# DeNA/HandyRL

Measured on NVIDIA H100. Metric: learner_samples_per_sec, higher is better.
Workload: dtype fp32

## Files before the change

handyrl_b200/csrc/gemm_kernel.cu:

```cuda
#include <cuda_runtime.h>
#include <stdint.h>
#include <string.h>

#define HRL_GEMM_KERNEL gemm_tf32x3_kernel
#define HRL_GEMM_BF16 false
#include "gemm_common.cuh"

static int g_gemm_debug = 0;
extern "C" void hrl_gemm_set_debug(int v) { g_gemm_debug = v; }

namespace hrl {

__global__ void sum_partials_kernel(const float *__restrict__ partials, int splits, long long n, long long stride, float *__restrict__ out) {
    for (long long i = (long long)blockIdx.x * blockDim.x + threadIdx.x; i < n; i += (long long)gridDim.x * blockDim.x) {
        float s = partials[i];
        for (int k = 1; k < splits; k++) s += partials[(long long)k * stride + i];
        out[i] = s;
    }
}

template <bool A_K, bool B_K, bool PACKED, int NW>
static int launch_gemm(const GemmParams &p, dim3 grid, size_t smem_bytes, cudaStream_t stream) {
    HRL_CUDA_CHECK(cudaFuncSetAttribute(gemm_tf32x3_kernel<A_K, B_K, PACKED, NW>, cudaFuncAttributeMaxDynamicSharedMemorySize, (int)smem_bytes));
    gemm_tf32x3_kernel<A_K, B_K, PACKED, NW><<<grid, kGemmThreads, smem_bytes, stream>>>(p);
    return HRL_OK;
}

template <int NW>
static int launch_gemm_width(const GemmParams &p, dim3 grid, size_t smem_bytes, cudaStream_t stream) {
    if (p.b.packed) return p.a.kmajor ? launch_gemm<true, true, true, NW>(p, grid, smem_bytes, stream)
                                      : launch_gemm<false, true, true, NW>(p, grid, smem_bytes, stream);
    if (p.a.kmajor) return p.b.kmajor ? launch_gemm<true, true, false, NW>(p, grid, smem_bytes, stream)
                                      : launch_gemm<true, false, false, NW>(p, grid, smem_bytes, stream);
    return p.b.kmajor ? launch_gemm<false, true, false, NW>(p, grid, smem_bytes, stream)
                      : launch_gemm<false, false, false, NW>(p, grid, smem_bytes, stream);
}

}


extern "C" size_t hrl_gemm_workspace_floats(int64_t M, int64_t N, int64_t K, int32_t splits) {
    (void)K;
    return splits > 1 ? (size_t)splits * (size_t)M * (size_t)N : 0;
}

extern "C" int32_t hrl_gemm_effective_splits(int64_t K, int32_t splits) {
    const int total_chunks = (int)((K + hrl::kChunkK - 1) / hrl::kChunkK);
    if (splits < 1) splits = 1;
    if (splits > total_chunks) splits = total_chunks;
    const int per = (total_chunks + splits - 1) / splits;
    return (total_chunks + per - 1) / per;
}

extern "C" int hrl_gemm_fused(const HrlGemmArgs *args, void *stream_) {
    using namespace hrl;
    cudaStream_t stream = reinterpret_cast<cudaStream_t>(stream_);
    HRL_REQUIRE(args != nullptr, HRL_ERR_BAD_ARG, "hrl_gemm_fused: args is NULL");
    const HrlGemmArgs &g = *args;
    const int64_t M = g.M, N = g.N, K = g.K;
    int splits = g.splits;
    HRL_REQUIRE(g.a.ptr && g.b.ptr && (g.C || ((splits > 1 || g.segments > 0) && g.workspace)), HRL_ERR_BAD_ARG, "hrl_gemm_fused: NULL pointer");
    HRL_REQUIRE(M > 0 && N > 0 && K > 0 && M < (1ll << 31) && N < (1ll << 22) && K < (1ll << 31) && g.b.ld < (1ll << 22), HRL_ERR_BAD_ARG,
                "hrl_gemm_fused: bad dimensions (M=%lld N=%lld K=%lld)", (long long)M, (long long)N, (long long)K);
    HRL_REQUIRE(g.conv_mode >= 0 && g.conv_mode <= 2, HRL_ERR_BAD_ARG, "hrl_gemm_fused: conv_mode is 0, 1 or 2");
    if (g.conv_mode != 0) {
        HRL_REQUIRE(g.conv_off && g.conv_hw > 0 && g.conv_taps > 0 && g.conv_cin > 0 && g.conv_cin < 65536 &&
                        (long long)g.conv_hw * g.conv_taps <= hrl::kConvMaxTable && g.a.p == nullptr && g.b.p == nullptr && g.splits >= 1,
                    HRL_ERR_BAD_ARG, "hrl_gemm_fused: convolution geometry (at most 256 cells x 9 taps, plain operands)");
        if (g.conv_mode == 1)
            HRL_REQUIRE(g.b.packed && g.a.kmajor && g.a.ld >= g.conv_cin && g.a.ld % 4 == 0 && (reinterpret_cast<uintptr_t>(g.a.ptr) & 15) == 0 &&
                            M % g.conv_hw == 0 && K == (int64_t)g.conv_taps * ((g.conv_cin + kChunkK - 1) / kChunkK) * kChunkK && g.splits == 1,
                        HRL_ERR_UNSUPPORTED,
                        "hrl_gemm_fused: convolution forward needs a packed B image over taps x (channels padded to 32), 16-byte aligned "
                        "pixel rows and whole boards");
        else
            HRL_REQUIRE(!g.b.packed && !g.a.kmajor && !g.b.kmajor && g.b.ld >= g.conv_cin &&
                            N == (int64_t)g.conv_taps * g.conv_cin + (g.conv_ones_row ? 1 : 0) && K % g.conv_hw == 0,
                        HRL_ERR_UNSUPPORTED,
                        "hrl_gemm_fused: convolution weight gradient reduces over whole boards of pixels, N = taps x channels (+ 1 with the ones row)");
    }
    HRL_REQUIRE(g.segments >= 0 && g.segments <= hrl::kMaxSegments &&
                    (g.segments == 0 || (g.conv_mode == 2 && g.seg_a && g.seg_b && g.workspace && g.C == nullptr)),
                HRL_ERR_BAD_ARG, "hrl_gemm_fused: up to %d segments, of a convolution weight gradient left as slice partials in the workspace",
                hrl::kMaxSegments);
    HRL_REQUIRE(!g.conv_ones_row || g.conv_mode == 2, HRL_ERR_BAD_ARG, "hrl_gemm_fused: the ones row belongs to the convolution weight gradient");
    HRL_REQUIRE((g.conv_mode == 1 || g.a.ld >= (g.a.kmajor ? K : M)) && (g.b.packed || g.conv_mode == 2 || g.b.ld >= (g.b.kmajor ? K : N)) &&
                    (g.C == nullptr || g.ldc >= N),
                HRL_ERR_BAD_ARG, "hrl_gemm_fused: leading dimension smaller than the row length");
    HRL_REQUIRE(!g.a.packed && (!g.b.packed || (N <= hrl::kMaxN && g.b.p == nullptr && (reinterpret_cast<uintptr_t>(g.b.ptr) & 15) == 0)),
                HRL_ERR_BAD_ARG, "hrl_gemm_fused: only an untransformed B operand of at most 288 rows can be a packed image");
    HRL_REQUIRE((g.a.p == nullptr) == (g.a.r == nullptr) && (g.b.p == nullptr) == (g.b.r == nullptr) &&
                    (g.a.ptr2 == nullptr || (g.a.p && g.a.q)) && (g.b.ptr2 == nullptr || (g.b.p && g.b.q)),
                HRL_ERR_BAD_ARG, "hrl_gemm_fused: an operand transform needs p and r (and q with a second source)");
    HRL_REQUIRE(g.epilogue >= HRL_GEMM_EP_STORE && g.epilogue <= HRL_GEMM_EP_MASK_STATS, HRL_ERR_BAD_ARG, "hrl_gemm_fused: unknown epilogue");
    HRL_REQUIRE(g.epilogue != HRL_GEMM_EP_MASK_STATS || (g.ep_y != nullptr && g.ep_ldy >= N && (g.ep_mean == nullptr) == (g.ep_rstd == nullptr)),
                HRL_ERR_BAD_ARG, "hrl_gemm_fused: the masked epilogue needs the pre-activation tile");
    HRL_REQUIRE(g.epilogue < HRL_GEMM_EP_STATS || (N % 4 == 0 && g.ldc % 4 == 0 && (reinterpret_cast<uintptr_t>(g.C) & 15) == 0 && g.col_partials),
                HRL_ERR_UNSUPPORTED, "hrl_gemm_fused: the statistics epilogues need N and ldc multiples of 4, a 16-byte aligned C and col_partials");
    const int total_chunks = (int)((K + kChunkK - 1) / kChunkK);
    if (splits < 1) splits = 1;
    if (splits > total_chunks) splits = total_chunks;
    HRL_REQUIRE((splits == 1 && g.segments == 0) || (g.workspace != nullptr && g.bias == nullptr && g.epilogue == HRL_GEMM_EP_STORE), HRL_ERR_WORKSPACE,
                "hrl_gemm_fused: a split-K product needs a workspace of hrl_gemm_workspace_floats() floats, no bias and the plain epilogue");
    const int n_tiles = (int)((N + kMaxN - 1) / kMaxN);
    const int n_widest = (int)(N < kMaxN ? N : kMaxN);
    int n_pad = (n_widest + 15) / 16 * 16;
    if (n_pad > 256) n_pad = (n_pad + 31) / 32 * 32;

    GemmParams p;
    auto operand = [](const HrlGemmOperand &o) {
        GemmOperand r;
        r.ptr = o.ptr; r.ptr2 = o.ptr2; r.p = o.p; r.q = o.q; r.r = o.r; r.ld = o.ld;
        r.kmajor = o.kmajor ? 1 : 0; r.relu = o.relu ? 1 : 0; r.feature_is_row = o.feature_is_row ? 1 : 0; r.packed = o.packed ? 1 : 0;
        return r;
    };
    p.a = operand(g.a);
    p.b = operand(g.b);
    p.bias = g.bias;
    p.M = (int)M; p.N = (int)N; p.K = (int)K;
    p.chunks_per_split = (total_chunks + splits - 1) / splits;
    p.epilogue = g.epilogue;
    p.ep_y = g.ep_y; p.ep_ldy = g.ep_ldy;
    p.ep_scale = g.ep_scale; p.ep_shift = g.ep_shift; p.ep_mean = g.ep_mean; p.ep_rstd = g.ep_rstd;
    p.col_partials = g.col_partials;
    p.debug = g_gemm_debug & 63;
    p.conv_off = g.conv_off; p.conv_mode = g.conv_mode; p.conv_hw = g.conv_hw; p.conv_taps = g.conv_taps; p.conv_cin = g.conv_cin;
    p.conv_cpt = (g.conv_cin + kChunkK - 1) / kChunkK;
    splits = (total_chunks + p.chunks_per_split - 1) / p.chunks_per_split;
    p.seg_splits = 0;
    p.conv_ones = g.conv_ones_row ? 1 : 0;
    if (g.segments > 0) {
        p.seg_splits = splits;
        for (int i = 0; i < g.segments; i++) { p.seg_a[i] = g.seg_a[i]; p.seg_b[i] = g.seg_b[i]; }
        splits *= g.segments;
    }
    if (splits > 1 || g.segments > 0) {
        p.C = g.workspace; p.ldc = N; p.c_split_stride = M * N;
    } else {
        p.C = g.C; p.ldc = g.ldc; p.c_split_stride = 0;
    }
    size_t smem_bytes = 1024 + (size_t)kStages * (g.bf16 ? ((size_t)n_pad + kTileM) * kChunkK * 2
                                                         : 2 * (size_t)n_pad * kChunkK * 4 + 2 * (size_t)kTileM * kChunkK * 4);
    const size_t red_rows = (size_t)kGemmThreads / (size_t)((n_pad - 12) / 4 > 0 ? (n_pad - 12) / 4 : 1);
    const size_t ep_bytes = 1024 + ((size_t)kTileM * (n_pad + 4) + 2 * red_rows * (size_t)n_pad) * 4;
    if (smem_bytes < ep_bytes) smem_bytes = ep_bytes;
    const dim3 grid((unsigned)((M + kTileM - 1) / kTileM), (unsigned)n_tiles, (unsigned)splits);
    int st;
    if (g.bf16) st = launch_gemm_bf16(p, n_pad / 2, grid, smem_bytes, stream);
    else switch (n_pad / 2) {
    case 8: st = launch_gemm_width<8>(p, grid, smem_bytes, stream); break;
    case 16: st = launch_gemm_width<16>(p, grid, smem_bytes, stream); break;
    case 24: st = launch_gemm_width<24>(p, grid, smem_bytes, stream); break;
    case 32: st = launch_gemm_width<32>(p, grid, smem_bytes, stream); break;
    case 40: st = launch_gemm_width<40>(p, grid, smem_bytes, stream); break;
    case 48: st = launch_gemm_width<48>(p, grid, smem_bytes, stream); break;
    case 56: st = launch_gemm_width<56>(p, grid, smem_bytes, stream); break;
    case 64: st = launch_gemm_width<64>(p, grid, smem_bytes, stream); break;
    case 72: st = launch_gemm_width<72>(p, grid, smem_bytes, stream); break;
    case 80: st = launch_gemm_width<80>(p, grid, smem_bytes, stream); break;
    case 88: st = launch_gemm_width<88>(p, grid, smem_bytes, stream); break;
    case 96: st = launch_gemm_width<96>(p, grid, smem_bytes, stream); break;
    case 104: st = launch_gemm_width<104>(p, grid, smem_bytes, stream); break;
    case 112: st = launch_gemm_width<112>(p, grid, smem_bytes, stream); break;
    case 120: st = launch_gemm_width<120>(p, grid, smem_bytes, stream); break;
    case 128: st = launch_gemm_width<128>(p, grid, smem_bytes, stream); break;
    case 144: st = launch_gemm_width<144>(p, grid, smem_bytes, stream); break;
    default: HRL_REQUIRE(false, HRL_ERR_BAD_ARG, "hrl_gemm_fused: no kernel for a tile of %d padded columns", n_pad);
    }
    if (st != HRL_OK) return st;
    HRL_CUDA_CHECK(cudaGetLastError());
    if (splits > 1 && g.C != nullptr) {
        const long long n = (long long)M * N;
        HRL_REQUIRE(g.ldc == N, HRL_ERR_UNSUPPORTED, "hrl_gemm_fused: split-K output must be dense (ldc == N)");
        int blocks = (int)((n + 255) / 256);
        if (blocks > 1184) blocks = 1184;
        sum_partials_kernel<<<blocks, 256, 0, stream>>>(g.workspace, splits, n, n, g.C);
        HRL_CUDA_CHECK(cudaGetLastError());
    }
    return HRL_OK;
}

extern "C" int hrl_gemm_tf32x3(const float *A, int64_t lda, int32_t a_kmajor, const float *B, int64_t ldb, int32_t b_kmajor,
                               const float *bias, float *C, int64_t ldc, int64_t M, int64_t N, int64_t K, int32_t splits,
                               float *workspace, void *stream) {
    HrlGemmArgs g;
    memset(&g, 0, sizeof(g));
    g.a.ptr = A; g.a.ld = lda; g.a.kmajor = a_kmajor;
    g.b.ptr = B; g.b.ld = ldb; g.b.kmajor = b_kmajor;
    g.bias = bias; g.C = C; g.ldc = ldc; g.M = M; g.N = N; g.K = K; g.splits = splits; g.workspace = workspace;
    g.epilogue = HRL_GEMM_EP_STORE;
    return hrl_gemm_fused(&g, stream);
}
```

Measured before the change: 19.29 million.

## Add specialized 3xTF32 weight-gradient GEMM kernel with larger tiles

Adds a dedicated weight-gradient GEMM kernel for M-major operands that uses 96x288 block tiles, 48x48 warp tiles, a three-stage cp.async pipeline, and conflict-free padded shared-memory strides. It applies the fused per-feature affine/ReLU transforms while loading fragments. Eligible GEMMs (fp32, no conv mode, no segments, plain store epilogue) are routed to it instead of the generic width-templated kernel. The aim is better data reuse and tensor-core throughput on wgrad shapes, at the cost of more code paths and a single-block-per-SM launch bound that may underfill the GPU on small problems.

After: 21.87 million (median of 6 runs). 1.13x the previous value.

```diff
diff --git a/handyrl_b200/csrc/gemm_kernel.cu b/handyrl_b200/csrc/gemm_kernel.cu
--- a/handyrl_b200/csrc/gemm_kernel.cu
+++ b/handyrl_b200/csrc/gemm_kernel.cu
@@ -5,6 +5,7 @@
 #define HRL_GEMM_KERNEL gemm_tf32x3_kernel
 #define HRL_GEMM_BF16 false
 #include "gemm_common.cuh"
+#include "gemm_wgrad.cuh"
 
 static int g_gemm_debug = 0;
 extern "C" void hrl_gemm_set_debug(int v) { g_gemm_debug = v; }
@@ -146,7 +147,8 @@
     if (smem_bytes < ep_bytes) smem_bytes = ep_bytes;
     const dim3 grid((unsigned)((M + kTileM - 1) / kTileM), (unsigned)n_tiles, (unsigned)splits);
     int st;
-    if (g.bf16) st = launch_gemm_bf16(p, n_pad / 2, grid, smem_bytes, stream);
+    if (gemm_wgrad_applies(g)) st = launch_gemm_wgrad(g, p.chunks_per_split, splits, p.C, p.ldc, p.c_split_stride, p.debug, stream);
+    else if (g.bf16) st = launch_gemm_bf16(p, n_pad / 2, grid, smem_bytes, stream);
     else switch (n_pad / 2) {
     case 8: st = launch_gemm_width<8>(p, grid, smem_bytes, stream); break;
     case 16: st = launch_gemm_width<16>(p, grid, smem_bytes, stream); break;
diff --git a/handyrl_b200/csrc/gemm_wgrad.cuh b/handyrl_b200/csrc/gemm_wgrad.cuh
--- /dev/null
+++ b/handyrl_b200/csrc/gemm_wgrad.cuh
@@ -0,0 +1,13 @@
+#pragma once
+#include <cuda_runtime.h>
+
+#include "common.cuh"
+
+namespace hrl {
+
+bool gemm_wgrad_applies(const HrlGemmArgs &g);
+
+int launch_gemm_wgrad(const HrlGemmArgs &g, int chunks_per_split, int splits, float *C, long long ldc, long long c_split_stride,
+                      int debug, cudaStream_t stream);
+
+}
diff --git a/handyrl_b200/csrc/gemm_wgrad_kernel.cu b/handyrl_b200/csrc/gemm_wgrad_kernel.cu
--- /dev/null
+++ b/handyrl_b200/csrc/gemm_wgrad_kernel.cu
@@ -0,0 +1,276 @@
+#include <cuda_runtime.h>
+#include <stdint.h>
+
+#include "gemm_wgrad.cuh"
+
+namespace hrl {
+namespace {
+
+constexpr int kThreads = 384;
+constexpr int kTileM = 96, kTileN = 288;
+constexpr int kWarpM = 48, kWarpN = 48;
+constexpr int kChunk = 32;
+constexpr int kStages = 3;
+constexpr int kLdA = kTileM + 8;
+constexpr int kLdB = kTileN + 8;
+constexpr int kStageFloats = 2 * kChunk * kLdA + kChunk * kLdB;
+constexpr size_t kSmemBytes = (size_t)kStages * kStageFloats * 4;
+static_assert(kLdA % 32 == 8 && kLdB % 32 == 8, "conflict-free fragment loads need row strides == 8 (mod 32) words");
+
+struct Operand {
+    const float *ptr, *ptr2;
+    const float *p, *q, *r;
+    long long ld;
+    int relu;
+};
+
+struct Params {
+    Operand a, b;
+    float *C;
+    long long ldc, c_split_stride;
+    int M, N, K, chunks_per_split;
+    int debug;
+};
+
+template <int KIND>
+__device__ __forceinline__ float transform(float x, float y, float p, float q, float r, bool relu) {
+    if (KIND == 0) return x;
+    const float v = KIND == 2 ? fmaf(x, p, fmaf(y, q, r)) : fmaf(x, p, r);
+    return relu ? fmaxf(v, 0.f) : v;
+}
+
+__device__ __forceinline__ void split(float v, uint32_t &hi, uint32_t &lo) {
+    hi = __float_as_uint(v) & 0xFFFFE000u;
+    lo = __float_as_uint(v - __uint_as_float(hi));
+}
+
+__device__ __forceinline__ void mma_tf32(float (&d)[4], const uint32_t (&a)[4], uint32_t b0, uint32_t b1) {
+    asm("mma.sync.aligned.m16n8k8.row.col.f32.tf32.tf32.f32 {%0, %1, %2, %3}, {%4, %5, %6, %7}, {%8, %9}, {%0, %1, %2, %3};"
+        : "+f"(d[0]), "+f"(d[1]), "+f"(d[2]), "+f"(d[3])
+        : "r"(a[0]), "r"(a[1]), "r"(a[2]), "r"(a[3]), "r"(b0), "r"(b1));
+}
+
+__device__ __forceinline__ void cp_async16(uint32_t dst, const float *src) {
+    asm volatile("cp.async.cg.shared.global [%0], [%1], 16;" ::"r"(dst), "l"(src) : "memory");
+}
+__device__ __forceinline__ void cp_async_commit() { asm volatile("cp.async.commit_group;" ::: "memory"); }
+template <int N>
+__device__ __forceinline__ void cp_async_wait() { asm volatile("cp.async.wait_group %0;" ::"n"(N) : "memory"); }
+
+template <int KIND, bool IS_A>
+__device__ __forceinline__ void load_consts(const Operand &op, int row0, int rows, float (&p)[6], float (&q)[6], float (&r)[6]) {
+#pragma unroll
+    for (int u = 0; u < 6; u++) {
+        const int row = row0 + 16 * (u >> 1) + (u & 1);
+        p[u] = q[u] = r[u] = 0.f;
+        if (KIND == 0 || row >= rows) continue;
+        p[u] = __ldg(op.p + row);
+        r[u] = __ldg(op.r + row);
+        if (op.q != nullptr) q[u] = __ldg(op.q + row);
+        if (KIND == 1 && IS_A) r[u] = fmaf(0.f, q[u], r[u]);
+    }
+}
+
+template <int AK, int BK, bool TAIL>
+__device__ __forceinline__ void mma_chunk(float (&acc)[3][6][4], const float *st, int mw, int nw, int g, int t, int k_left,
+                                          const float (&pa)[6], const float (&qa)[6], const float (&ra)[6], bool relu_a,
+                                          const float (&pb)[6], const float (&qb)[6], const float (&rb)[6], bool relu_b) {
+    const float *sa = st, *sa2 = st + kChunk * kLdA, *sb = st + 2 * kChunk * kLdA;
+#pragma unroll
+    for (int ks = 0; ks < kChunk / 8; ks++) {
+        const int k0 = 8 * ks + t, k1 = k0 + 4;
+        const bool v0 = !TAIL || k0 < k_left, v1 = !TAIL || k1 < k_left;
+        uint32_t ahi[3][4], alo[3][4];
+#pragma unroll
+        for (int i = 0; i < 3; i++) {
+            const int m = mw + 16 * i + 2 * g;
+            const float2 x0 = *reinterpret_cast<const float2 *>(sa + k0 * kLdA + m);
+            const float2 x1 = *reinterpret_cast<const float2 *>(sa + k1 * kLdA + m);
+            float2 y0 = make_float2(0.f, 0.f), y1 = y0;
+            if (AK == 2) {
+                y0 = *reinterpret_cast<const float2 *>(sa2 + k0 * kLdA + m);
+                y1 = *reinterpret_cast<const float2 *>(sa2 + k1 * kLdA + m);
+            }
+            const int u = 2 * i;
+            float v[4] = {transform<AK>(x0.x, y0.x, pa[u], qa[u], ra[u], relu_a), transform<AK>(x0.y, y0.y, pa[u + 1], qa[u + 1], ra[u + 1], relu_a),
+                          transform<AK>(x1.x, y1.x, pa[u], qa[u], ra[u], relu_a), transform<AK>(x1.y, y1.y, pa[u + 1], qa[u + 1], ra[u + 1], relu_a)};
+            if (TAIL) {
+                if (!v0) v[0] = v[1] = 0.f;
+                if (!v1) v[2] = v[3] = 0.f;
+            }
+#pragma unroll
+            for (int e = 0; e < 4; e++) split(v[e], ahi[i][e], alo[i][e]);
+        }
+#pragma unroll
+        for (int jp = 0; jp < 3; jp++) {
+            const int n = nw + 16 * jp + 2 * g;
+            const float2 z0 = *reinterpret_cast<const float2 *>(sb + k0 * kLdB + n);
+            const float2 z1 = *reinterpret_cast<const float2 *>(sb + k1 * kLdB + n);
+            const int u = 2 * jp;
+            float v[2][2] = {{transform<BK>(z0.x, 0.f, pb[u], qb[u], rb[u], relu_b), transform<BK>(z1.x, 0.f, pb[u], qb[u], rb[u], relu_b)},
+                             {transform<BK>(z0.y, 0.f, pb[u + 1], qb[u + 1], rb[u + 1], relu_b),
+                              transform<BK>(z1.y, 0.f, pb[u + 1], qb[u + 1], rb[u + 1], relu_b)}};
+            if (TAIL) {
+                if (!v0) v[0][0] = v[1][0] = 0.f;
+                if (!v1) v[0][1] = v[1][1] = 0.f;
+            }
+            uint32_t bhi[2][2], blo[2][2];
+#pragma unroll
+            for (int j = 0; j < 2; j++)
+#pragma unroll
+                for (int h = 0; h < 2; h++) split(v[j][h], bhi[j][h], blo[j][h]);
+#pragma unroll
+            for (int i = 0; i < 3; i++)
+#pragma unroll
+                for (int j = 0; j < 2; j++) mma_tf32(acc[i][2 * jp + j], alo[i], bhi[j][0], bhi[j][1]);
+#pragma unroll
+            for (int i = 0; i < 3; i++)
+#pragma unroll
+                for (int j = 0; j < 2; j++) mma_tf32(acc[i][2 * jp + j], ahi[i], blo[j][0], blo[j][1]);
+#pragma unroll
+            for (int i = 0; i < 3; i++)
+#pragma unroll
+                for (int j = 0; j < 2; j++) mma_tf32(acc[i][2 * jp + j], ahi[i], bhi[j][0], bhi[j][1]);
+        }
+    }
+}
+
+template <int AK, int BK>
+__global__ void __launch_bounds__(kThreads, 1) gemm_wgrad_kernel(const Params p) {
+    extern __shared__ __align__(16) float smem[];
+    const int tid = threadIdx.x, warp = tid >> 5, lane = tid & 31, g = lane >> 2, t = lane & 3;
+    const int m0 = blockIdx.x * kTileM, n0 = blockIdx.y * kTileN, split = blockIdx.z;
+    const int mw = (warp & 1) * kWarpM, nw = (warp >> 1) * kWarpN;
+    const bool active = m0 + mw < p.M && n0 + nw < p.N;
+    const int total_chunks = (p.K + kChunk - 1) / kChunk;
+    const int c_begin = split * p.chunks_per_split, c_end = min(total_chunks, c_begin + p.chunks_per_split);
+
+    float pa[6], qa[6], ra[6], pb[6], qb[6], rb[6];
+    load_consts<AK, true>(p.a, m0 + mw + 2 * g, p.M, pa, qa, ra);
+    load_consts<BK, false>(p.b, n0 + nw + 2 * g, p.N, pb, qb, rb);
+    const bool relu_a = AK != 0 && p.a.relu, relu_b = BK != 0 && p.b.relu;
+
+    const uint32_t smem_base = (uint32_t)__cvta_generic_to_shared(smem);
+    auto issue = [&](int c, int s) {
+        if (c < c_end && (p.debug & 3) != 2) {
+            const int k0 = c * kChunk;
+            const uint32_t st = smem_base + (uint32_t)s * kStageFloats * 4;
+            constexpr int kGroupsA = kTileM / 4, kGroupsB = kTileN / 4;
+#pragma unroll
+            for (int u = 0; u < kChunk * kGroupsA / kThreads; u++) {
+                const int i = tid + u * kThreads, k = i / kGroupsA, col = 4 * (i - k * kGroupsA);
+                if (k0 + k < p.K && m0 + col < p.M) {
+                    const long long off = (long long)(k0 + k) * p.a.ld + m0 + col;
+                    const uint32_t dst = st + (uint32_t)(k * kLdA + col) * 4;
+                    cp_async16(dst, p.a.ptr + off);
+                    if (AK == 2) cp_async16(dst + kChunk * kLdA * 4, p.a.ptr2 + off);
+                }
+            }
+#pragma unroll
+            for (int u = 0; u < kChunk * kGroupsB / kThreads; u++) {
+                const int i = tid + u * kThreads, k = i / kGroupsB, col = 4 * (i - k * kGroupsB);
+                if (k0 + k < p.K && n0 + col < p.N)
+                    cp_async16(st + (uint32_t)(2 * kChunk * kLdA + k * kLdB + col) * 4, p.b.ptr + (long long)(k0 + k) * p.b.ld + n0 + col);
+            }
+        }
+        cp_async_commit();
+    };
+
+    float acc[3][6][4];
+#pragma unroll
+    for (int i = 0; i < 3; i++)
+#pragma unroll
+        for (int j = 0; j < 6; j++)
+#pragma unroll
+            for (int e = 0; e < 4; e++) acc[i][j][e] = 0.f;
+
+#pragma unroll
+    for (int s = 0; s < kStages - 1; s++) issue(c_begin + s, s);
+    for (int c = c_begin; c < c_end; c++) {
+        const int it = c - c_begin;
+        cp_async_wait<kStages - 2>();
+        __syncthreads();
+        issue(c + kStages - 1, (it + kStages - 1) % kStages);
+        if (active && (p.debug & 3) != 1) {
+            const float *st = smem + (it % kStages) * kStageFloats;
+            const int k_left = p.K - c * kChunk;
+            if (k_left >= kChunk)
+                mma_chunk<AK, BK, false>(acc, st, mw, nw, g, t, k_left, pa, qa, ra, relu_a, pb, qb, rb, relu_b);
+            else
+                mma_chunk<AK, BK, true>(acc, st, mw, nw, g, t, k_left, pa, qa, ra, relu_a, pb, qb, rb, relu_b);
+        }
+    }
+    cp_async_wait<0>();
+
+    if (!active) return;
+    float *Cg = p.C + (long long)split * p.c_split_stride;
+    const bool vec = (p.ldc % 4 == 0) && ((reinterpret_cast<uintptr_t>(Cg) & 15) == 0);
+#pragma unroll
+    for (int i = 0; i < 3; i++) {
+#pragma unroll
+        for (int h = 0; h < 2; h++) {
+            const int m = m0 + mw + 16 * i + 2 * g + h;
+            if (m >= p.M) continue;
+            float *row = Cg + (long long)m * p.ldc;
+#pragma unroll
+            for (int jp = 0; jp < 3; jp++) {
+                const int n = n0 + nw + 16 * jp + 4 * t;
+                const float v[4] = {acc[i][2 * jp][2 * h], acc[i][2 * jp + 1][2 * h], acc[i][2 * jp][2 * h + 1], acc[i][2 * jp + 1][2 * h + 1]};
+                if (vec && n + 3 < p.N) {
+                    *reinterpret_cast<float4 *>(row + n) = make_float4(v[0], v[1], v[2], v[3]);
+                } else {
+#pragma unroll
+                    for (int e = 0; e < 4; e++)
+                        if (n + e < p.N) row[n + e] = v[e];
+                }
+            }
+        }
+    }
+}
+
+template <int AK, int BK>
+int launch(const Params &p, dim3 grid, cudaStream_t stream) {
+    HRL_CUDA_CHECK(cudaFuncSetAttribute(gemm_wgrad_kernel<AK, BK>, cudaFuncAttributeMaxDynamicSharedMemorySize, (int)kSmemBytes));
+    gemm_wgrad_kernel<AK, BK><<<grid, kThreads, kSmemBytes, stream>>>(p);
+    return HRL_OK;
+}
+
+template <int AK>
+int launch_b(const Params &p, int bk, dim3 grid, cudaStream_t stream) {
+    return bk == 0 ? launch<AK, 0>(p, grid, stream) : launch<AK, 1>(p, grid, stream);
+}
+
+bool aligned16(const void *ptr) { return (reinterpret_cast<uintptr_t>(ptr) & 15) == 0; }
+
+int kind_of(const HrlGemmOperand &o) { return o.p == nullptr ? 0 : o.ptr2 == nullptr ? 1 : 2; }
+
+}
+
+bool gemm_wgrad_applies(const HrlGemmArgs &g) {
+    auto fits = [](const HrlGemmOperand &o) {
+        return !o.kmajor && !o.packed && (o.p == nullptr || o.feature_is_row) && o.ld % 4 == 0 && aligned16(o.ptr) &&
+               (o.ptr2 == nullptr || aligned16(o.ptr2));
+    };
+    return !g.bf16 && g.conv_mode == 0 && g.segments == 0 && g.epilogue == HRL_GEMM_EP_STORE && g.bias == nullptr && fits(g.a) &&
+           fits(g.b) && g.b.ptr2 == nullptr;
+}
+
+int launch_gemm_wgrad(const HrlGemmArgs &g, int chunks_per_split, int splits, float *C, long long ldc, long long c_split_stride,
+                      int debug, cudaStream_t stream) {
+    Params p;
+    auto operand = [](const HrlGemmOperand &o) {
+        Operand r;
+        r.ptr = o.ptr; r.ptr2 = o.ptr2; r.p = o.p; r.q = o.q; r.r = o.r; r.ld = o.ld; r.relu = o.relu ? 1 : 0;
+        return r;
+    };
+    p.a = operand(g.a);
+    p.b = operand(g.b);
+    p.C = C; p.ldc = ldc; p.c_split_stride = c_split_stride;
+    p.M = (int)g.M; p.N = (int)g.N; p.K = (int)g.K; p.chunks_per_split = chunks_per_split;
+    p.debug = debug;
+    const dim3 grid((unsigned)((g.M + kTileM - 1) / kTileM), (unsigned)((g.N + kTileN - 1) / kTileN), (unsigned)splits);
+    const int ak = kind_of(g.a), bk = kind_of(g.b);
+    return ak == 0 ? launch_b<0>(p, bk, grid, stream) : ak == 1 ? launch_b<1>(p, bk, grid, stream) : launch_b<2>(p, bk, grid, stream);
+}
+
+}
```
